# BUBLET/uav-airvision

Hardware: AMD Instinct MI355X
Metric: stereo frames/sec (LK+stereo+MSCKF-update) at 752x480 (higher is better)
Workload: dtype u8/int32 windows, f32 normal equations

## Files before the change

### uav_airvision_amd/csrc/lk.hip

```cpp
#include <math.h>
#include <stdio.h>
#include <stdlib.h>

#include "av_common.h"

namespace {

struct LKArgs {
    const uint8_t* pyrI;
    const uint8_t* pyrJ;
    int64_t stream_stride;
    PyrGeom g;
    const float* prev;
    float* next;
    uint8_t* status;
    const int* count;
    const int* index;
    int cap;
    int max_iter;
    double eps2;
    float min_eig_up, eps_lo, eps_hi;
    double min_eig;
    int n_set, gx;
    const uint8_t* imgI; const uint8_t* imgJ;
    int64_t imgI_stride, imgJ_stride;
    const int* mapI; const int* mapJ;
    unsigned long long* prof;
};

enum { LKP_HEAD = 0, LKP_ISTAGE, LKP_SETUP, LKP_JSTAGE, LKP_ITER, LKP_N, LKP_WAVES = LKP_N, LKP_ITERS, LKP_RESTAGES, LKP_LEVELS, LKP_SLOTS };

__device__ __forceinline__ void wave_lds_sync()
{
    __builtin_amdgcn_fence(__ATOMIC_RELEASE, "wavefront");
    __builtin_amdgcn_wave_barrier();
    __builtin_amdgcn_fence(__ATOMIC_ACQUIRE, "wavefront");
}

#define AV_DESCALE(x, n) (((x) + (1 << ((n)-1))) >> (n))

typedef short av_v2s __attribute__((ext_vector_type(2)));
__device__ __forceinline__ int dot2(uint32_t a, uint32_t b, int c)
{
    return __builtin_amdgcn_sdot2(__builtin_bit_cast(av_v2s, a), __builtin_bit_cast(av_v2s, b), c, false);
}
__device__ __forceinline__ int dot2_keep(uint32_t a, uint32_t b, int c)
{
    int r;
    asm("v_dot2_i32_i16 %0, %1, %2, %3" : "=v"(r) : "v"(a), "v"(b), "v"(c));
    return r;
}
__device__ __forceinline__ uint32_t pack16(int lo, int hi) { return ((uint32_t)lo & 0xFFFFu) | ((uint32_t)hi << 16); }

constexpr int TILE_ROWS = 24;
constexpr int TILE_COLS = 32;
constexpr int TPITCH = 36;
constexpr int TILE_DWORDS = 240;

typedef unsigned short av_v2u __attribute__((ext_vector_type(2)));

__device__ __forceinline__ uint32_t pk_add(uint32_t a, uint32_t b) { return __builtin_bit_cast(uint32_t, __builtin_bit_cast(av_v2u, a) + __builtin_bit_cast(av_v2u, b)); }
__device__ __forceinline__ uint32_t pk_sub(uint32_t a, uint32_t b) { return __builtin_bit_cast(uint32_t, __builtin_bit_cast(av_v2u, a) - __builtin_bit_cast(av_v2u, b)); }
__device__ __forceinline__ uint32_t pk_mul(uint32_t a, unsigned short k) { av_v2u kk = {k, k}; return __builtin_bit_cast(uint32_t, __builtin_bit_cast(av_v2u, a) * kk); }
// ... 160 lines not shown
        const bool rowin = (unsigned)(ipy + r) < (unsigned)h;
#pragma unroll
        for (int k = 0; k < 8; ++k) {
            const uint32_t m0 = (rowin && (unsigned)(ipx_o + 2 * k) < (unsigned)w) ? 0xFFFFu : 0u;
            const uint32_t m1 = (rowin && (unsigned)(ipx_o + 2 * k + 1) < (unsigned)w) ? 0xFFFF0000u : 0u;
            gxp[2 * k] &= (m0 | m1); gyp[2 * k] &= (m0 | m1);
        }
    }
#pragma unroll
    for (int k = 0; k < 7; ++k) {
        gxp[2 * k + 1] = mid(gxp[2 * k], gxp[2 * k + 2]);
        gyp[2 * k + 1] = mid(gyp[2 * k], gyp[2 * k + 2]);
    }
    const int rnd_i = 1 << (W_BITS - 6), rnd_d = 1 << (W_BITS - 1);
    int ixv[WIN + 1], iyv[WIN + 1];
    ixv[WIN] = 0; iyv[WIN] = 0;
#pragma unroll
    for (int c = 0; c < WIN; c += 5) {
        bilin5_seed(px[c], px[c + 1], px[c + 2], px[c + 3], px[c + 4], wtop, wbot, rnd_i, iv[c], iv[c + 1], iv[c + 2], iv[c + 3], iv[c + 4]);
        bilin5<W_BITS>(gxp[c], gxp[c + 1], gxp[c + 2], gxp[c + 3], gxp[c + 4], wtop, wbot, rnd_d, ixv[c], ixv[c + 1], ixv[c + 2], ixv[c + 3], ixv[c + 4]);
        bilin5<W_BITS>(gyp[c], gyp[c + 1], gyp[c + 2], gyp[c + 3], gyp[c + 4], wtop, wbot, rnd_d, iyv[c], iyv[c + 1], iyv[c + 2], iyv[c + 3], iyv[c + 4]);
    }
#pragma unroll
    for (int p = 0; p < (WIN + 1) / 2; ++p) {
        ixx[p] = __builtin_amdgcn_perm((uint32_t)ixv[2 * p + 1], (uint32_t)ixv[2 * p], 0x05040100u);
        iyy[p] = __builtin_amdgcn_perm((uint32_t)iyv[2 * p + 1], (uint32_t)iyv[2 * p], 0x05040100u);
        a11 = dot2(ixx[p], ixx[p], a11);
        a12 = dot2(ixx[p], iyy[p], a12);
        a22 = dot2(iyy[p], iyy[p], a22);
    }
    if (r >= WIN) { a11 = 0; a12 = 0; a22 = 0; }
}

template <int WIN, int OCC, bool PROF = false, int PTS = 16>
__device__ __forceinline__ bool lk_track_g16_body(const LKArgs& a)
{
    static_assert(WIN == 15, "lane map is built for the reference's 15x15 window");
    constexpr int W_BITS = 14;
    __shared__ uint32_t tile_all[PTS][TILE_DWORDS];
    unsigned pt[LKP_N] = {0, 0, 0, 0, 0}, plast = 0;
    unsigned pn_iter = 0, pn_restage = 0, pn_level = 0;
    unsigned long long rt0 = 0;
    if (PROF) { rt0 = __builtin_amdgcn_s_memrealtime(); plast = (unsigned)__builtin_readcyclecounter(); }
#define LK_STAMP(ph) do { if (PROF) { const unsigned t_ = (unsigned)__builtin_readcyclecounter(); pt[ph] += t_ - plast; plast = t_; } } while (0)
    const int g = threadIdx.x >> 4;
    const int r = threadIdx.x & 15;
    uint32_t* tile = tile_all[g];
    int s, bx;
    if (a.gx > 0) { const int L = blockIdx.x, j = L >> 3; s = (L & 7) + 8 * (j / a.gx); bx = j % a.gx; if (s >= a.n_set) return false; }
    else { s = blockIdx.y; bx = blockIdx.x; }
    const int slot = bx * PTS + g;
    const int sI = a.mapI ? a.mapI[s] : s, sJ = a.mapJ ? a.mapJ[s] : s;
    if (sI < 0 || sJ < 0) return false;
    const bool direct = a.index == nullptr && slot < a.cap;
    float prevx0 = 0.f, prevy0 = 0.f, curx = 0.f, cury = 0.f;
    if (direct) {
        const size_t p0 = (size_t)s * a.cap + slot;
        prevx0 = a.prev[2 * p0]; prevy0 = a.prev[2 * p0 + 1]; curx = a.next[2 * p0]; cury = a.next[2 * p0 + 1];
    }
    const int n = min(a.count[s], a.cap);
    if (slot >= n) return false;
    const int pidx = a.index ? a.index[(size_t)s * a.cap + slot] : slot;

    const uint8_t* PI = a.pyrI + sI * a.stream_stride;
    const uint8_t* PJ = a.pyrJ + sJ * a.stream_stride;
    const size_t pi = (size_t)s * a.cap + pidx;
    if (!direct) { prevx0 = a.prev[2 * pi]; prevy0 = a.prev[2 * pi + 1]; curx = a.next[2 * pi]; cury = a.next[2 * pi + 1]; }
    const float halfWin = (WIN - 1) * 0.5f;
    const bool rowact = r < WIN;
    bool ok = true;
    const uint32_t sel0 = 0x0C010C00u, sel1 = 0x0C020C01u, sel2 = 0x0C030C02u, sel3 = 0x0C040C03u;

    for (int level = a.g.levels - 1; level >= 0; --level) {
        const int w = a.g.w[level], h = a.g.h[level], pitch = a.g.pitch[level];
        const int col_lo = -AV_PYR_BORDER, col_hi = pitch - AV_PYR_BORDER;
        const float scale = __int_as_float((127 - level) << 23);
        float pvx = prevx0 * scale, pvy = prevy0 * scale;
        if (level == a.g.levels - 1) { curx = curx * scale; cury = cury * scale; }
        else                         { curx = curx * 2.f;   cury = cury * 2.f; }
        pvx -= halfWin; pvy -= halfWin;
        const int ipx = (int)floorf(pvx), ipy = (int)floorf(pvy);
        if (ipx < -WIN || ipx >= w || ipy < -WIN || ipy >= h) {
            if (level == 0) ok = false;
            continue;
        }
        float fa = pvx - ipx, fb = pvy - ipy;
        int iw00 = __float2int_rn((1.f - fa) * (1.f - fb) * (1 << W_BITS));
        int iw01 = __float2int_rn(fa * (1.f - fb) * (1 << W_BITS));
        int iw10 = __float2int_rn((1.f - fa) * fb * (1 << W_BITS));
        int iw11 = (1 << W_BITS) - iw00 - iw01 - iw10;
        uint32_t wtop = pack16(iw00, iw01), wbot = pack16(iw10, iw11);

        const int sub = r >> 3, dwl = r & 7;
        const uint32_t tofs = (uint32_t)(sub * (TPITCH / 4) + dwl);
// ... 26 lines not shown
                    uint32_t v = 0;
#pragma unroll 1
                    for (int bb = 0; bb < nbyte; ++bb) v |= (uint32_t)row[av_reflect101(xb + bb, w)] << (8 * bb);
                    tile[tofs + 2 * k * (TPITCH / 4)] = v;
                }
            }
        }
        wave_lds_sync();
        LK_STAMP(LKP_ISTAGE);

        int iv[WIN];
        uint32_t ixx[(WIN + 1) / 2], iyy[(WIN + 1) / 2];
        int a11, a12, a22;
        lk_patch_rows<WIN>([&](int t, uint32_t (&B)[5]) {
                               const uint32_t* rowp = tile + __mul24(r + t, TPITCH / 4);
#pragma unroll
                               for (int k = 0; k < 5; ++k) B[k] = rowp[k];
                           }, wtop, wbot, ipx, ipy, w, h, r, iv, ixx, iyy, a11, a12, a22);
        const float A11 = row_sum16_scaled(a11);
        const float A12 = row_sum16_scaled(a12);
        const float A22 = row_sum16_scaled(a22);
        float D = A11 * A22 - A12 * A12;
        const float minEig = (A22 + A11 - sqrtf((A11 - A22) * (A11 - A22) + 4.f * A12 * A12)) / (float)(2 * WIN * WIN);
        if (minEig < a.min_eig_up || D < 1.1920928955078125e-7f) {
            if (level == 0) ok = false;
            continue;
        }
        D = 1.f / D;

        float wx = curx - halfWin, wy = cury - halfWin;
        float pdx = 0.f, pdy = 0.f;
        int X0 = 0, Y0 = 0;
        bool staged = false;
        LK_STAMP(LKP_SETUP);
        for (int j = 0; j < a.max_iter; ++j) {
            if (PROF) ++pn_iter;
            const int inx = (int)floorf(wx), iny = (int)floorf(wy);
            if (inx < -WIN || inx >= w || iny < -WIN || iny >= h) {
                if (level == 0) ok = false;
                break;
            }
            int dx0 = inx - X0, dy0 = iny - Y0;
            if (!staged || (unsigned)dx0 > (unsigned)(TILE_COLS - 17) || (unsigned)dy0 > (unsigned)(TILE_ROWS - 16)) {
                X0 = min(max((inx - 6) & ~3, col_lo), col_hi - TILE_COLS);
                Y0 = min(max(iny - 4, -AV_PYR_BORDER), h + AV_PYR_BORDER - TILE_ROWS);
                LK_STAMP(LKP_ITER);
                if (PROF) ++pn_restage;
                wave_lds_sync();
                {
                    const bool extJ = level == 0 && a.imgJ != nullptr;
                    const uint8_t* LJ0 = extJ ? a.imgJ + (size_t)sJ * (size_t)a.imgJ_stride : PJ + a.g.off[level];
                    const int pJ = extJ ? w : pitch, bJ = extJ ? 0 : AV_PYR_BORDER;
                    if (!extJ || (X0 >= 0 && X0 + TILE_COLS <= w && Y0 >= 0 && Y0 + TILE_ROWS <= h)) {
                        const uint32_t joff = (uint32_t)(__mul24(Y0 + sub + bJ, pJ) + X0 + bJ + 4 * dwl);
                        uint32_t sv[TILE_ROWS / 2];
#pragma unroll
                        for (int k = 0; k < TILE_ROWS / 2; ++k)
                            sv[k] = *reinterpret_cast<const u32_unaligned*>(LJ0 + (size_t)(2 * k) * (size_t)pJ + joff);
#pragma unroll
                        for (int k = 0; k < TILE_ROWS / 2; ++k) tile[tofs + 2 * k * (TPITCH / 4)] = sv[k];
                    } else {
#pragma unroll 1
                        for (int k = 0; k < TILE_ROWS / 2; ++k) {
                            const uint8_t* row = LJ0 + (size_t)av_reflect101(Y0 + sub + 2 * k, h) * (size_t)w;
                            uint32_t v = 0;
#pragma unroll 1
// ... 21 lines not shown
            const uint32_t T2 = __builtin_amdgcn_alignbyte(d3, d2, sh), T3 = __builtin_amdgcn_alignbyte(d4, d3, sh);
            int df[WIN];
            jdiff5<0>(T0, T1, T2, T3, sel0, sel1, sel2, sel3, wtop, wbot, iv[0], iv[1], iv[2], iv[3], iv[4], df[0], df[1], df[2], df[3], df[4]);
            jdiff5<5>(T0, T1, T2, T3, sel0, sel1, sel2, sel3, wtop, wbot, iv[5], iv[6], iv[7], iv[8], iv[9], df[5], df[6], df[7], df[8], df[9]);
            jdiff5<10>(T0, T1, T2, T3, sel0, sel1, sel2, sel3, wtop, wbot, iv[10], iv[11], iv[12], iv[13], iv[14], df[10], df[11], df[12], df[13], df[14]);
            int b1 = 0, b2 = 0;
#pragma unroll
            for (int p = 0; p < (WIN + 1) / 2; ++p) {
                const uint32_t dp = 2 * p + 1 < WIN ? __builtin_amdgcn_perm((uint32_t)df[2 * p + 1 < WIN ? 2 * p + 1 : 0], (uint32_t)df[2 * p], 0x05040100u) : (uint32_t)df[2 * p];
                b1 = dot2(dp, ixx[p], b1);
                b2 = dot2(dp, iyy[p], b2);
            }
            if (!rowact) { b1 = 0; b2 = 0; }
            const float fb1 = row_sum16_scaled(b1);
            const float fb2 = row_sum16_scaled(b2);
            const float dx = (A12 * fb2 - A22 * fb1) * D;
            const float dy = (A12 * fb1 - A11 * fb2) * D;
            wx += dx; wy += dy;
            curx = wx + halfWin; cury = wy + halfWin;
            const float e32 = __builtin_fmaf(dx, dx, dy * dy);
            bool conv = e32 <= a.eps_lo;
            if (__builtin_amdgcn_ballot_w64(e32 > a.eps_lo && e32 < a.eps_hi) != 0) {
                asm volatile("; fp64 step test");
                conv = (double)dx * dx + (double)dy * dy <= a.eps2;
            }
            if (conv) break;
            if (j > 0 && fabsf(dx + pdx) <= 0.01f && fabsf(dy + pdy) <= 0.01f) {
                curx -= dx * 0.5f; cury -= dy * 0.5f;
                break;
            }
            pdx = dx; pdy = dy;
        }
        LK_STAMP(LKP_ITER);
    }
    if (r == 0) {
        a.next[2 * pi] = curx;
        a.next[2 * pi + 1] = cury;
        a.status[pi] = ok ? 1 : 0;
    }
    if (PROF) {
        LK_STAMP(LKP_HEAD);
        unsigned wi = pn_iter, wr = pn_restage, wl = pn_level;
#pragma unroll
        for (int d = 16; d < 64; d <<= 1) { wi = max(wi, (unsigned)__shfl_xor((int)wi, d, 64)); wr = max(wr, (unsigned)__shfl_xor((int)wr, d, 64)); wl = max(wl, (unsigned)__shfl_xor((int)wl, d, 64)); }
        const bool book = blockIdx.x % 61 == 0;
        if (book && (threadIdx.x & 63) == 0) {
            for (int k = 0; k < LKP_N; ++k) atomicAdd(a.prof + k, (unsigned long long)pt[k]);
            atomicAdd(a.prof + LKP_WAVES, 1ull);
            atomicAdd(a.prof + LKP_SLOTS + 3, __builtin_amdgcn_s_memrealtime() - rt0);
            atomicAdd(a.prof + LKP_ITERS, (unsigned long long)wi);
            atomicAdd(a.prof + LKP_RESTAGES, (unsigned long long)wr);
            atomicAdd(a.prof + LKP_LEVELS, (unsigned long long)wl);
        }
        if (book && r == 0) { atomicAdd(a.prof + LKP_SLOTS, 1ull); atomicAdd(a.prof + LKP_SLOTS + 1, (unsigned long long)pn_iter); atomicAdd(a.prof + LKP_SLOTS + 2, (unsigned long long)pn_restage); }
    }
#undef LK_STAMP
    return true;
}

template <int WIN> __global__ __launch_bounds__(64, 5) void lk_track_g16_kernel(LKArgs a) { lk_track_g16_body<WIN, 5, false, 4>(a); }
template <int WIN> __global__ __launch_bounds__(256, 5) void lk_track_g16_w4_kernel(LKArgs a) { lk_track_g16_body<WIN, 5>(a); }
template <int WIN> __global__ __launch_bounds__(256, 5) void lk_track_g16_prof_kernel(LKArgs a) { lk_track_g16_body<WIN, 5, true>(a); }

static unsigned long long* g_lk_prof = nullptr;
static void lk_prof_report()
{
    if (!g_lk_prof) return;
    unsigned long long h[LKP_SLOTS + 4];
    if (hipDeviceSynchronize() != hipSuccess || hipMemcpy(h, g_lk_prof, sizeof(h), hipMemcpyDeviceToHost) != hipSuccess) return;
    static const char* names[LKP_N] = {"head+tail", "I staging", "set-up", "J staging", "iterations"};
    double tot = 0;
    for (int k = 0; k < LKP_N; ++k) tot += (double)h[k];
    const double nw = (double)h[LKP_WAVES];
    fprintf(stderr, "AV_LK_PROF: %.0f wavefronts booked (one workgroup in 61), %.0f s_memtime ticks per wavefront = %.1f us on the 100 MHz clock: %.0f ticks per us\n",
            nw, tot / nw, (double)h[LKP_SLOTS + 3] / nw / 100., tot / ((double)h[LKP_SLOTS + 3] / 100.));
    for (int k = 0; k < LKP_N; ++k) fprintf(stderr, "AV_LK_PROF:   %-10s %8.0f ticks per wavefront  %5.1f %%\n", names[k], (double)h[k] / nw, 100. * (double)h[k] / tot);
    fprintf(stderr, "AV_LK_PROF: per wavefront (max over its 4 points): %.2f levels, %.2f iterations, %.2f J stagings; per point: %.2f iterations, %.2f J stagings\n",
            (double)h[LKP_LEVELS] / nw, (double)h[LKP_ITERS] / nw, (double)h[LKP_RESTAGES] / nw,
            (double)h[LKP_SLOTS + 1] / (double)h[LKP_SLOTS], (double)h[LKP_SLOTS + 2] / (double)h[LKP_SLOTS]);
}


constexpr int LKG_MAX_WIN = 31, LKG_PER_LANE = (LKG_MAX_WIN * LKG_MAX_WIN + 63) / 64;

__device__ __forceinline__ long long wave_sum_i64(long long v)
{
#pragma unroll
    for (int d = 32; d >= 1; d >>= 1) v += __shfl_xor(v, d, 64);
    return v;
}

struct LKLevel { const uint8_t* base; int pitch, w, h; };
__device__ __forceinline__ int lkg_pix(const LKLevel& L, int x, int y) { return L.base[(size_t)av_reflect101_any(y, L.h) * L.pitch + av_reflect101_any(x, L.w)]; }

__global__ __launch_bounds__(256) void lk_track_generic_kernel(LKArgs a, int WIN)
{
    constexpr int W_BITS = 14;
    const int lane = threadIdx.x & 63;
    const int s = blockIdx.y, slot = blockIdx.x * 4 + (threadIdx.x >> 6);
    const int sI = a.mapI ? a.mapI[s] : s, sJ = a.mapJ ? a.mapJ[s] : s;
    if (sI < 0 || sJ < 0) return;
    const int n = min(a.count[s], a.cap);
    if (slot >= n) return;
    const int pidx = a.index ? a.index[(size_t)s * a.cap + slot] : slot;
    const size_t pi = (size_t)s * a.cap + pidx;
    const float prevx0 = a.prev[2 * pi], prevy0 = a.prev[2 * pi + 1];
    float curx = a.next[2 * pi], cury = a.next[2 * pi + 1];
    const float halfWin = (WIN - 1) * 0.5f;
    const int win2 = WIN * WIN;
    const double FLT_SCALE_D = 1.0 / (1 << 20);
    bool ok = true;
    for (int level = a.g.levels - 1; level >= 0; --level) {
// ... 106 lines not shown
        a.next[2 * pi + 1] = cury;
        a.status[pi] = ok ? 1 : 0;
    }
}

}

static int lk_fill_args(LKArgs& a, const uint8_t* pyrI, const uint8_t* pyrJ, int64_t stream_stride, const PyrGeom& g,
                        const float* prev, float* next, uint8_t* status, const int* count, int cap,
                        const LKParams& p, const int* index,
                        const uint8_t* imgI, int64_t imgI_stride, const uint8_t* imgJ, int64_t imgJ_stride, const int* mapI, const int* mapJ)
{
    if (p.win < 3 || p.win > LKG_MAX_WIN) { av_set_error("av_lk_track: winSize %d outside 3 .. %d", p.win, LKG_MAX_WIN); return AV_E_INVALID; }
    a.pyrI = pyrI; a.pyrJ = pyrJ; a.stream_stride = stream_stride; a.g = g;
    for (int l = 1; l < a.g.levels; ++l)
        if (a.g.w[l] <= p.win || a.g.h[l] <= p.win) { a.g.levels = l; break; }
    a.prev = prev; a.next = next; a.status = status; a.count = count; a.index = index; a.cap = cap;
    a.max_iter = p.max_iter; a.eps2 = p.eps2;
    a.min_eig_up = (float)p.min_eig;
    if ((double)a.min_eig_up < p.min_eig) a.min_eig_up = nextafterf(a.min_eig_up, INFINITY);
    if (p.eps2 >= 1e-30) { a.eps_lo = (float)(p.eps2 * (1. - 0x1p-18)); a.eps_hi = (float)(p.eps2 * (1. + 0x1p-18)); }
    else { a.eps_lo = -1.f; a.eps_hi = INFINITY; }
    a.min_eig = p.min_eig;
    a.imgI = imgI; a.imgJ = imgJ; a.imgI_stride = imgI_stride; a.imgJ_stride = imgJ_stride; a.mapI = mapI; a.mapJ = mapJ; a.prof = nullptr;
    a.n_set = 0; a.gx = 0;
    return AV_OK;
}

static bool lk_prof_on()
{
    static const bool prof = [] {
        const char* e = getenv("AV_LK_PROF");
        if (!(e && atoi(e) == 1)) return false;
        if (hipMalloc(&g_lk_prof, sizeof(unsigned long long) * (LKP_SLOTS + 4)) != hipSuccess) { g_lk_prof = nullptr; return false; }
        (void)hipMemset(g_lk_prof, 0, sizeof(unsigned long long) * (LKP_SLOTS + 4));
        (void)hipDeviceSynchronize();
        atexit(lk_prof_report);
        return true;
    }();
    return prof;
}

static dim3 lk_g16_grid(LKArgs& a, int n_set, int launch_pts, int pts_per_wg)
{
    static const bool xcd_map = [] { const char* e = getenv("AV_LK_XCD"); return !(e && atoi(e) == 0); }();
    const int gx = (launch_pts + pts_per_wg - 1) / pts_per_wg;
    a.n_set = n_set; a.gx = xcd_map ? gx : 0;
    return xcd_map ? dim3((unsigned)gx * 8u * (unsigned)((n_set + 7) / 8)) : dim3(gx, n_set);
}

int av_launch_lk(const uint8_t* pyrI, const uint8_t* pyrJ, int64_t stream_stride, int n_set, const PyrGeom& g,
                 const float* prev, float* next, uint8_t* status, const int* count, int cap, int launch_pts,
                 const LKParams& p, hipStream_t st, const int* index,
                 const uint8_t* imgI, int64_t imgI_stride, const uint8_t* imgJ, int64_t imgJ_stride, const int* mapI, const int* mapJ)
{
    if (n_set <= 0 || launch_pts <= 0) return AV_OK;
    LKArgs a;
    int rc = lk_fill_args(a, pyrI, pyrJ, stream_stride, g, prev, next, status, count, cap, p, index, imgI, imgI_stride, imgJ, imgJ_stride, mapI, mapJ);
    if (rc) return rc;
    if (launch_pts > cap) launch_pts = cap;
    if (p.win != 15) {
        a.n_set = n_set; a.gx = 0;
        hipLaunchKernelGGL(lk_track_generic_kernel, dim3((launch_pts + 3) / 4, n_set), dim3(256), 0, st, a, p.win);
        AV_LAUNCH_CHECK();
        return AV_OK;
    }
    const bool prof = lk_prof_on();
    static const bool w1 = [] { const char* e = getenv("AV_LK_WG"); return !(e && atoi(e) == 256); }();
    const int wgp = (prof || !w1) ? 256 : 64;
    const dim3 grid = lk_g16_grid(a, n_set, launch_pts, wgp / 16);
    a.prof = g_lk_prof;
    if (prof) hipLaunchKernelGGL(lk_track_g16_prof_kernel<15>, grid, dim3(256), 0, st, a);
    else if (wgp == 64) hipLaunchKernelGGL(lk_track_g16_kernel<15>, grid, dim3(64), 0, st, a);
    else hipLaunchKernelGGL(lk_track_g16_w4_kernel<15>, grid, dim3(256), 0, st, a);
    AV_LAUNCH_CHECK();
    return AV_OK;
}

AV_EXPORT int av_lk_track(const uint8_t* pyrI_dev, const uint8_t* pyrJ_dev, int64_t pyr_stride, int n_set,
                          int w, int h, int levels,
                          const float* prev_dev, float* next_dev, uint8_t* status_dev, const int32_t* count_dev, int cap,
                          int win, int max_iter, double eps, double min_eig_threshold, void* stream)
{
    av_pyr_layout lay;
    int rc = av_pyramid_layout(w, h, levels, &lay);
    if (rc) return rc;
    if (!pyrI_dev || !pyrJ_dev || !prev_dev || !next_dev || !status_dev || !count_dev || cap <= 0 || n_set < 0 ||
        pyr_stride < lay.bytes) {
        av_set_error("av_lk_track: bad arguments");
        return AV_E_INVALID;
    }
    LKParams p;
    p.win = win;
    p.max_iter = max_iter < 0 ? 0 : (max_iter > 100 ? 100 : max_iter);
    double e = eps < 0 ? 0. : (eps > 10. ? 10. : eps);
    p.eps2 = e * e;
    p.min_eig = min_eig_threshold;
    return av_launch_lk(pyrI_dev, pyrJ_dev, pyr_stride, n_set, av_make_geom(lay), prev_dev, next_dev, status_dev,
                        count_dev, cap, cap, p, (hipStream_t)stream, nullptr);
}
// ... 1 lines not shown
```

Before: 200,400.

## Track each LK point with 8 lanes handling two window rows each

After: 198,800 (median of 2 runs). No clear change (-0.8%).

```diff
diff --git a/uav_airvision_amd/csrc/lk.hip b/uav_airvision_amd/csrc/lk.hip
--- a/uav_airvision_amd/csrc/lk.hip
+++ b/uav_airvision_amd/csrc/lk.hip
@@ -29,6 +29,8 @@
 };
 
 enum { LKP_HEAD = 0, LKP_ISTAGE, LKP_SETUP, LKP_JSTAGE, LKP_ITER, LKP_N, LKP_WAVES = LKP_N, LKP_ITERS, LKP_RESTAGES, LKP_LEVELS, LKP_SLOTS };
+enum { LKP_DIV4 = LKP_SLOTS + 4, LKP_NDIV4, LKP_DIV8, LKP_NDIV8, LKP_WORDS };
+constexpr int LKD_G4 = 8, LKD_G8 = 4, LKD_WORDS = (LKD_G4 + LKD_G8) * (AV_MAX_LEVELS + 1);
 
 __device__ __forceinline__ void wave_lds_sync()
 {
@@ -255,8 +257,39 @@
     if (r >= WIN) { a11 = 0; a12 = 0; a22 = 0; }
 }
 
+__device__ __forceinline__ void lk_div_active(unsigned* lvm, int g)
+{
+    atomicMax(lvm + (LKD_G4 + LKD_G8) * AV_MAX_LEVELS + (g >> 2), 1u);
+    atomicMax(lvm + (LKD_G4 + LKD_G8) * AV_MAX_LEVELS + LKD_G4 + (g >> 3), 1u);
+}
+__device__ __forceinline__ void lk_div_level(unsigned* lvm, int g, int level, unsigned iters)
+{
+    atomicMax(lvm + (g >> 2) * AV_MAX_LEVELS + level, iters);
+    atomicMax(lvm + (LKD_G4 + (g >> 3)) * AV_MAX_LEVELS + level, iters);
+}
+__device__ __forceinline__ void lk_div_init(unsigned* lvm)
+{
+    for (int i = threadIdx.x; i < LKD_WORDS; i += blockDim.x) lvm[i] = 0;
+    __syncthreads();
+}
+__device__ __forceinline__ void lk_div_book(const LKArgs& a, const unsigned* lvm)
+{
+    __syncthreads();
+    if (threadIdx.x != 0 || blockIdx.x % 61 != 0) return;
+    unsigned long long it[2] = {0, 0}, ng[2] = {0, 0};
+    for (int k = 0; k < 2; ++k)
+        for (int grp = 0; grp < (k ? LKD_G8 : LKD_G4); ++grp) {
+            const int row = (k ? LKD_G4 : 0) + grp;
+            if (!lvm[(LKD_G4 + LKD_G8) * AV_MAX_LEVELS + row]) continue;
+            ++ng[k];
+            for (int l = 0; l < AV_MAX_LEVELS; ++l) it[k] += lvm[row * AV_MAX_LEVELS + l];
+        }
+    atomicAdd(a.prof + LKP_DIV4, it[0]); atomicAdd(a.prof + LKP_NDIV4, ng[0]);
+    atomicAdd(a.prof + LKP_DIV8, it[1]); atomicAdd(a.prof + LKP_NDIV8, ng[1]);
+}
+
 template <int WIN, int OCC, bool PROF = false, int PTS = 16>
-__device__ __forceinline__ bool lk_track_g16_body(const LKArgs& a)
+__device__ __forceinline__ bool lk_track_g16_body(const LKArgs& a, unsigned* lvm = nullptr)
 {
     static_assert(WIN == 15, "lane map is built for the reference's 15x15 window");
     constexpr int W_BITS = 14;
@@ -283,6 +316,7 @@
     }
     const int n = min(a.count[s], a.cap);
     if (slot >= n) return false;
+    if (PROF && r == 0) lk_div_active(lvm, g);
     const int pidx = a.index ? a.index[(size_t)s * a.cap + slot] : slot;
 
     const uint8_t* PI = a.pyrI + sI * a.stream_stride;
@@ -375,6 +409,7 @@
         float pdx = 0.f, pdy = 0.f;
         int X0 = 0, Y0 = 0;
         bool staged = false;
+        const unsigned it_lv0 = pn_iter;
         LK_STAMP(LKP_SETUP);
         for (int j = 0; j < a.max_iter; ++j) {
             if (PROF) ++pn_iter;
@@ -462,6 +497,7 @@
             pdx = dx; pdy = dy;
         }
         LK_STAMP(LKP_ITER);
+        if (PROF && r == 0) lk_div_level(lvm, g, level, pn_iter - it_lv0);
     }
     if (r == 0) {
         a.next[2 * pi] = curx;
@@ -490,13 +526,438 @@
 
 template <int WIN> __global__ __launch_bounds__(64, 5) void lk_track_g16_kernel(LKArgs a) { lk_track_g16_body<WIN, 5, false, 4>(a); }
 template <int WIN> __global__ __launch_bounds__(256, 5) void lk_track_g16_w4_kernel(LKArgs a) { lk_track_g16_body<WIN, 5>(a); }
-template <int WIN> __global__ __launch_bounds__(256, 5) void lk_track_g16_prof_kernel(LKArgs a) { lk_track_g16_body<WIN, 5, true>(a); }
+template <int WIN> __global__ __launch_bounds__(256, 5) void lk_track_g16_prof_kernel(LKArgs a)
+{
+    __shared__ unsigned lvm[LKD_WORDS];
+    lk_div_init(lvm);
+    lk_track_g16_body<WIN, 5, true>(a, lvm);
+    lk_div_book(a, lvm);
+}
+
+constexpr int G8_TILE_DWORDS = 216;
+
+__device__ __forceinline__ float row_sum8_scaled(int v)
+{
+    v += __builtin_amdgcn_update_dpp(0, v, 0xB1, 0xF, 0xF, false);
+    int lo = v & 0xFFFF, hi = v >> 16;
+    lo += __builtin_amdgcn_update_dpp(0, lo, 0x4E, 0xF, 0xF, false);
+    hi += __builtin_amdgcn_update_dpp(0, hi, 0x4E, 0xF, 0xF, false);
+    lo += __builtin_amdgcn_update_dpp(0, lo, 0x141, 0xF, 0xF, false);
+    hi += __builtin_amdgcn_update_dpp(0, hi, 0x141, 0xF, 0xF, false);
+    return __builtin_fmaf((float)hi, 0x1p-4f, (float)lo * 0x1p-20f);
+}
+
+#define AV_G8_BILIN(X) AV_G8_BILIN_(X)
+#define AV_G8_BILIN_(BOT, TAIL)                                                                                                   \
+    "v_dot2_i32_i16 %0, %5, %15, %17\n\t" "v_dot2_i32_i16 %1, %6, %15, %17\n\t" "v_dot2_i32_i16 %2, %7, %15, %17\n\t"            \
+    "v_dot2_i32_i16 %3, %8, %15, %17\n\t" "v_dot2_i32_i16 %4, %9, %15, %17\n\t"                                                   \
+    "v_dot2c_i32_i16" BOT " %0, %10, %16" TAIL "\n\t" "v_dot2c_i32_i16" BOT " %1, %11, %16" TAIL "\n\t"                           \
+    "v_dot2c_i32_i16" BOT " %2, %12, %16" TAIL "\n\t" "v_dot2c_i32_i16" BOT " %3, %13, %16" TAIL "\n\t"                           \
+    "v_dot2c_i32_i16" BOT " %4, %14, %16" TAIL "\n\t"
+#define AV_G8_DPP "_dpp", " row_shl:1 row_mask:0xf bank_mask:0xf bound_ctrl:1"
+#define AV_G8_OWN "", ""
+template <int SH, bool NB>
+__device__ __forceinline__ void bilin5_2(const uint32_t* t, const uint32_t* b, uint32_t wtop, uint32_t wbot, int rnd, int* o)
+{
+#define AV_G8_SHIFT "v_ashrrev_i32 %0, %18, %0\n\tv_ashrrev_i32 %1, %18, %1\n\tv_ashrrev_i32 %2, %18, %2\n\tv_ashrrev_i32 %3, %18, %3\n\tv_ashrrev_i32 %4, %18, %4"
+#define AV_G8_ARGS : "=&v"(o[0]), "=&v"(o[1]), "=&v"(o[2]), "=&v"(o[3]), "=&v"(o[4]) \
+                   : "v"(t[0]), "v"(t[1]), "v"(t[2]), "v"(t[3]), "v"(t[4]), "v"(b[0]), "v"(b[1]), "v"(b[2]), "v"(b[3]), "v"(b[4]), \
+                     "v"(wtop), "v"(wbot), "v"(rnd)
+    if (NB) asm(AV_G8_BILIN(AV_G8_DPP) AV_G8_SHIFT AV_G8_ARGS, "n"(SH));
+    else    asm(AV_G8_BILIN(AV_G8_OWN) AV_G8_SHIFT AV_G8_ARGS, "n"(SH));
+#undef AV_G8_SHIFT
+}
+template <bool NB>
+__device__ __forceinline__ void bilin5_2_seed(const uint32_t* t, const uint32_t* b, uint32_t wtop, uint32_t wbot, int rnd, int* o)
+{
+#define AV_G8_SEED "v_and_b32 %0, %18, %0\n\tv_and_b32 %1, %18, %1\n\tv_and_b32 %2, %18, %2\n\tv_and_b32 %3, %18, %3\n\tv_and_b32 %4, %18, %4\n\t" \
+                   "v_sub_u32 %0, %19, %0\n\tv_sub_u32 %1, %19, %1\n\tv_sub_u32 %2, %19, %2\n\tv_sub_u32 %3, %19, %3\n\tv_sub_u32 %4, %19, %4"
+    if (NB) asm(AV_G8_BILIN(AV_G8_DPP) AV_G8_SEED AV_G8_ARGS, "s"(0xfffffe00u), "s"(0x100u));
+    else    asm(AV_G8_BILIN(AV_G8_OWN) AV_G8_SEED AV_G8_ARGS, "s"(0xfffffe00u), "s"(0x100u));
+#undef AV_G8_SEED
+}
+template <bool NB>
+__device__ __forceinline__ void jdot5_2(const uint32_t* t, const uint32_t* b, uint32_t wtop, uint32_t wbot, const int* s, int* d)
+{
+#define AV_G8_JD(X) AV_G8_JD_(X)
+#define AV_G8_JD_(BOT, TAIL)                                                                                                     \
+    "v_dot2_i32_i16 %0, %5, %15, %17\n\t" "v_dot2_i32_i16 %1, %6, %15, %18\n\t" "v_dot2_i32_i16 %2, %7, %15, %19\n\t"            \
+    "v_dot2_i32_i16 %3, %8, %15, %20\n\t" "v_dot2_i32_i16 %4, %9, %15, %21\n\t"                                                   \
+    "v_dot2c_i32_i16" BOT " %0, %10, %16" TAIL "\n\t" "v_dot2c_i32_i16" BOT " %1, %11, %16" TAIL "\n\t"                           \
+    "v_dot2c_i32_i16" BOT " %2, %12, %16" TAIL "\n\t" "v_dot2c_i32_i16" BOT " %3, %13, %16" TAIL "\n\t"                           \
+    "v_dot2c_i32_i16" BOT " %4, %14, %16" TAIL "\n\t"                                                                             \
+    "v_ashrrev_i32 %0, 9, %0\n\tv_ashrrev_i32 %1, 9, %1\n\tv_ashrrev_i32 %2, 9, %2\n\tv_ashrrev_i32 %3, 9, %3\n\tv_ashrrev_i32 %4, 9, %4"
+#define AV_G8_JARGS : "=&v"(d[0]), "=&v"(d[1]), "=&v"(d[2]), "=&v"(d[3]), "=&v"(d[4]) \
+                    : "v"(t[0]), "v"(t[1]), "v"(t[2]), "v"(t[3]), "v"(t[4]), "v"(b[0]), "v"(b[1]), "v"(b[2]), "v"(b[3]), "v"(b[4]), \
+                      "v"(wtop), "v"(wbot), "v"(s[0]), "v"(s[1]), "v"(s[2]), "v"(s[3]), "v"(s[4])
+    if (NB) asm(AV_G8_JD(AV_G8_DPP) AV_G8_JARGS);
+    else    asm(AV_G8_JD(AV_G8_OWN) AV_G8_JARGS);
+#undef AV_G8_JD
+#undef AV_G8_JD_
+#undef AV_G8_JARGS
+}
+#undef AV_G8_ARGS
+#undef AV_G8_BILIN
+#undef AV_G8_BILIN_
+#undef AV_G8_DPP
+#undef AV_G8_OWN
+
+template <int WIN>
+__device__ __forceinline__ void lk_patch_rows2(const uint32_t* rowp, uint32_t wtop, uint32_t wbot, uint32_t wtopB, uint32_t wbotB,
+                                               int ipx, int ipy, int w, int h, int q,
+                                               int (&ivA)[WIN], uint32_t (&ixxA)[(WIN + 1) / 2], uint32_t (&iyyA)[(WIN + 1) / 2],
+                                               int (&ivB)[WIN], uint32_t (&ixxB)[(WIN + 1) / 2], uint32_t (&iyyB)[(WIN + 1) / 2],
+                                               int& a11, int& a12, int& a22)
+{
+    constexpr int W_BITS = 14;
+    uint32_t E[4][9];
+#pragma unroll
+    for (int t = 0; t < 4; ++t) {
+        uint32_t B[5];
+#pragma unroll
+        for (int k = 0; k < 5; ++k) B[k] = rowp[t * (TPITCH / 4) + k];
+#pragma unroll
+        for (int k = 0; k < 9; ++k) {
+            const int b0 = 2 * k;
+            E[t][k] = __builtin_amdgcn_perm(0, B[b0 >> 2], 0x0C000C00u | (uint32_t)(b0 & 3) | ((uint32_t)((b0 & 3) + 1) << 16));
+        }
+    }
+    auto mid = [](uint32_t x, uint32_t y) -> uint32_t { return __builtin_amdgcn_perm(y, x, 0x05040302u); };
+    uint32_t pxA[WIN], pxB[WIN];
+#pragma unroll
+    for (int k = 0; k < 8; ++k) { pxA[2 * k] = mid(E[1][k], E[1][k + 1]); pxB[2 * k] = mid(E[2][k], E[2][k + 1]); }
+#pragma unroll
+    for (int k = 0; k < 7; ++k) { pxA[2 * k + 1] = E[1][k + 1]; pxB[2 * k + 1] = E[2][k + 1]; }
+    uint32_t gxA[WIN + 1], gyA[WIN + 1], gxB[WIN + 1], gyB[WIN + 1];
+#pragma unroll
+    for (int rr = 0; rr < 2; ++rr) {
+        uint32_t* gxp = rr ? gxB : gxA;
+        uint32_t* gyp = rr ? gyB : gyA;
+        uint32_t t0E[9], t1E[9];
+#pragma unroll
+        for (int k = 0; k < 9; ++k) {
+            t0E[k] = pk_add(pk_mul(pk_add(E[rr][k], E[rr + 2][k]), 3), pk_mul(E[rr + 1][k], 10));
+            t1E[k] = pk_sub(E[rr + 2][k], E[rr][k]);
+        }
+#pragma unroll
+        for (int k = 0; k < 8; ++k) {
+            gxp[2 * k] = pk_sub(t0E[k + 1], t0E[k]);
+            gyp[2 * k] = pk_add(pk_mul(pk_add(t1E[k + 1], t1E[k]), 3), pk_mul(mid(t1E[k], t1E[k + 1]), 10));
+        }
+    }
+    const bool inside = ipx >= 0 && ipx + WIN < w && ipy >= 0 && ipy + WIN < h;
+    if (__builtin_amdgcn_ballot_w64(!inside) != 0) {
+        int ipx_o = ipx;
+        asm volatile("" : "+v"(ipx_o));
+#pragma unroll
+        for (int rr = 0; rr < 2; ++rr) {
+            uint32_t* gxp = rr ? gxB : gxA;
+            uint32_t* gyp = rr ? gyB : gyA;
+            const bool rowin = (unsigned)(ipy + 2 * q + rr) < (unsigned)h;
+#pragma unroll
+            for (int k = 0; k < 8; ++k) {
+                const uint32_t m0 = (rowin && (unsigned)(ipx_o + 2 * k) < (unsigned)w) ? 0xFFFFu : 0u;
+                const uint32_t m1 = (rowin && (unsigned)(ipx_o + 2 * k + 1) < (unsigned)w) ? 0xFFFF0000u : 0u;
+                gxp[2 * k] &= (m0 | m1); gyp[2 * k] &= (m0 | m1);
+            }
+        }
+    }
+#pragma unroll
+    for (int k = 0; k < 7; ++k) {
+        gxA[2 * k + 1] = mid(gxA[2 * k], gxA[2 * k + 2]); gyA[2 * k + 1] = mid(gyA[2 * k], gyA[2 * k + 2]);
+        gxB[2 * k + 1] = mid(gxB[2 * k], gxB[2 * k + 2]); gyB[2 * k + 1] = mid(gyB[2 * k], gyB[2 * k + 2]);
+    }
+    const int rnd_i = 1 << (W_BITS - 6), rnd_d = 1 << (W_BITS - 1);
+    int ixA[WIN + 1], iyA[WIN + 1], ixB[WIN + 1], iyB[WIN + 1];
+    ixA[WIN] = 0; iyA[WIN] = 0; ixB[WIN] = 0; iyB[WIN] = 0;
+#pragma unroll
+    for (int c = 0; c < WIN; c += 5) {
+        bilin5_2_seed<false>(pxA + c, pxB + c, wtop, wbot, rnd_i, ivA + c);
+        bilin5_2_seed<true>(pxB + c, pxA + c, wtopB, wbotB, rnd_i, ivB + c);
+        bilin5_2<W_BITS, false>(gxA + c, gxB + c, wtop, wbot, rnd_d, ixA + c);
+        bilin5_2<W_BITS, true>(gxB + c, gxA + c, wtopB, wbotB, rnd_d, ixB + c);
+        bilin5_2<W_BITS, false>(gyA + c, gyB + c, wtop, wbot, rnd_d, iyA + c);
+        bilin5_2<W_BITS, true>(gyB + c, gyA + c, wtopB, wbotB, rnd_d, iyB + c);
+    }
+    a11 = 0; a12 = 0; a22 = 0;
+#pragma unroll
+    for (int p = 0; p < (WIN + 1) / 2; ++p) {
+        ixxA[p] = __builtin_amdgcn_perm((uint32_t)ixA[2 * p + 1], (uint32_t)ixA[2 * p], 0x05040100u);
+        iyyA[p] = __builtin_amdgcn_perm((uint32_t)iyA[2 * p + 1], (uint32_t)iyA[2 * p], 0x05040100u);
+        ixxB[p] = __builtin_amdgcn_perm((uint32_t)ixB[2 * p + 1], (uint32_t)ixB[2 * p], 0x05040100u);
+        iyyB[p] = __builtin_amdgcn_perm((uint32_t)iyB[2 * p + 1], (uint32_t)iyB[2 * p], 0x05040100u);
+        a11 = dot2(ixxA[p], ixxA[p], a11); a12 = dot2(ixxA[p], iyyA[p], a12); a22 = dot2(iyyA[p], iyyA[p], a22);
+        a11 = dot2(ixxB[p], ixxB[p], a11); a12 = dot2(ixxB[p], iyyB[p], a12); a22 = dot2(iyyB[p], iyyB[p], a22);
+    }
+}
+
+template <int WIN, bool PROF = false, int PTS = 8>
+__device__ __forceinline__ bool lk_track_g8_body(const LKArgs& a, unsigned* lvm = nullptr)
+{
+    static_assert(WIN == 15, "lane map is built for the reference's 15x15 window");
+    constexpr int W_BITS = 14;
+    __shared__ uint32_t tile_all[PTS][G8_TILE_DWORDS];
+    unsigned pt[LKP_N] = {0, 0, 0, 0, 0}, plast = 0;
+    unsigned pn_iter = 0, pn_restage = 0, pn_level = 0;
+    unsigned long long rt0 = 0;
+    if (PROF) { rt0 = __builtin_amdgcn_s_memrealtime(); plast = (unsigned)__builtin_readcyclecounter(); }
+#define LK_STAMP(ph) do { if (PROF) { const unsigned t_ = (unsigned)__builtin_readcyclecounter(); pt[ph] += t_ - plast; plast = t_; } } while (0)
+    const int g = threadIdx.x >> 3;
+    const int q = threadIdx.x & 7;
+    uint32_t* tile = tile_all[g];
+    int s, bx;
+    if (a.gx > 0) { const int L = blockIdx.x, j = L >> 3; s = (L & 7) + 8 * (j / a.gx); bx = j % a.gx; if (s >= a.n_set) return false; }
+    else { s = blockIdx.y; bx = blockIdx.x; }
+    const int slot = bx * PTS + g;
+    const int sI = a.mapI ? a.mapI[s] : s, sJ = a.mapJ ? a.mapJ[s] : s;
+    if (sI < 0 || sJ < 0) return false;
+    const bool direct = a.index == nullptr && slot < a.cap;
+    float prevx0 = 0.f, prevy0 = 0.f, curx = 0.f, cury = 0.f;
+    if (direct) {
+        const size_t p0 = (size_t)s * a.cap + slot;
+        prevx0 = a.prev[2 * p0]; prevy0 = a.prev[2 * p0 + 1]; curx = a.next[2 * p0]; cury = a.next[2 * p0 + 1];
+    }
+    const int n = min(a.count[s], a.cap);
+    if (slot >= n) return false;
+    if (PROF && q == 0) lk_div_active(lvm, g);
+    const int pidx = a.index ? a.index[(size_t)s * a.cap + slot] : slot;
+
+    const uint8_t* PI = a.pyrI + sI * a.stream_stride;
+    const uint8_t* PJ = a.pyrJ + sJ * a.stream_stride;
+    const size_t pi = (size_t)s * a.cap + pidx;
+    if (!direct) { prevx0 = a.prev[2 * pi]; prevy0 = a.prev[2 * pi + 1]; curx = a.next[2 * pi]; cury = a.next[2 * pi + 1]; }
+    const float halfWin = (WIN - 1) * 0.5f;
+    const bool rowBin = q < 7;
+    bool ok = true;
+    const uint32_t sel0 = 0x0C010C00u, sel1 = 0x0C020C01u, sel2 = 0x0C030C02u, sel3 = 0x0C040C03u;
+    typedef uint32_t __attribute__((aligned(1))) u32_unaligned;
+
+    for (int level = a.g.levels - 1; level >= 0; --level) {
+        const int w = a.g.w[level], h = a.g.h[level], pitch = a.g.pitch[level];
+        const int col_lo = -AV_PYR_BORDER, col_hi = pitch - AV_PYR_BORDER;
+        const float scale = __int_as_float((127 - level) << 23);
+        float pvx = prevx0 * scale, pvy = prevy0 * scale;
+        if (level == a.g.levels - 1) { curx = curx * scale; cury = cury * scale; }
+        else                         { curx = curx * 2.f;   cury = cury * 2.f; }
+        pvx -= halfWin; pvy -= halfWin;
+        const int ipx = (int)floorf(pvx), ipy = (int)floorf(pvy);
+        if (ipx < -WIN || ipx >= w || ipy < -WIN || ipy >= h) {
+            if (level == 0) ok = false;
+            continue;
+        }
+        float fa = pvx - ipx, fb = pvy - ipy;
+        int iw00 = __float2int_rn((1.f - fa) * (1.f - fb) * (1 << W_BITS));
+        int iw01 = __float2int_rn(fa * (1.f - fb) * (1 << W_BITS));
+        int iw10 = __float2int_rn((1.f - fa) * fb * (1 << W_BITS));
+        int iw11 = (1 << W_BITS) - iw00 - iw01 - iw10;
+        uint32_t wtop = pack16(iw00, iw01), wbot = pack16(iw10, iw11);
+
+        LK_STAMP(LKP_HEAD);
+        if (PROF) ++pn_level;
+        wave_lds_sync();
+        {
+            const bool extI = level == 0 && a.imgI != nullptr;
+            const uint8_t* L0 = extI ? a.imgI + (size_t)sI * (size_t)a.imgI_stride : PI + a.g.off[level];
+            const int pI = extI ? w : pitch, bI = extI ? 0 : AV_PYR_BORDER;
+            const bool act = q < 5;
+            if (!extI || (ipx >= 1 && ipx + 16 < w && ipy >= 1 && ipy + 16 < h)) {
+                const uint32_t loff = (uint32_t)(__mul24(ipy - 1 + bI, pI) + (ipx - 1 + bI) + (q < 4 ? 4 * q : 14));
+                const uint32_t shamt = q == 4 ? 16u : 0u;
+                uint32_t sv[18];
+#pragma unroll
+                for (int k = 0; k < 18; ++k) {
+                    sv[k] = 0;
+                    if (act) sv[k] = *reinterpret_cast<const u32_unaligned*>(L0 + (size_t)k * (size_t)pI + loff);
+                }
+#pragma unroll
+                for (int k = 0; k < 18; ++k)
+                    if (act) tile[q + k * (TPITCH / 4)] = sv[k] >> shamt;
+            } else if (act) {
+                const int xb = ipx - 1 + (q < 4 ? 4 * q : 16), nbyte = q < 4 ? 4 : 2;
+#pragma unroll 1
+                for (int k = 0; k < 18; ++k) {
+                    const uint8_t* row = L0 + (size_t)av_reflect101(ipy - 1 + k, h) * (size_t)w;
+                    uint32_t v = 0;
+#pragma unroll 1
+                    for (int bb = 0; bb < nbyte; ++bb) v |= (uint32_t)row[av_reflect101(xb + bb, w)] << (8 * bb);
+                    tile[q + k * (TPITCH / 4)] = v;
+                }
+            }
+        }
+        wave_lds_sync();
+        LK_STAMP(LKP_ISTAGE);
+
+        int ivA[WIN], ivB[WIN];
+        uint32_t ixxA[(WIN + 1) / 2], iyyA[(WIN + 1) / 2], ixxB[(WIN + 1) / 2], iyyB[(WIN + 1) / 2];
+        int a11, a12, a22;
+        lk_patch_rows2<WIN>(tile + 2 * q * (TPITCH / 4), wtop, wbot, rowBin ? wtop : 0u, rowBin ? wbot : 0u, ipx, ipy, w, h, q,
+                            ivA, ixxA, iyyA, ivB, ixxB, iyyB, a11, a12, a22);
+        const float A11 = row_sum8_scaled(a11);
+        const float A12 = row_sum8_scaled(a12);
+        const float A22 = row_sum8_scaled(a22);
+        float D = A11 * A22 - A12 * A12;
+        const float minEig = (A22 + A11 - sqrtf((A11 - A22) * (A11 - A22) + 4.f * A12 * A12)) / (float)(2 * WIN * WIN);
+        if (minEig < a.min_eig_up || D < 1.1920928955078125e-7f) {
+            if (level == 0) ok = false;
+            continue;
+        }
+        D = 1.f / D;
+
+        float wx = curx - halfWin, wy = cury - halfWin;
+        float pdx = 0.f, pdy = 0.f;
+        int X0 = 0, Y0 = 0;
+        bool staged = false;
+        const unsigned it_lv0 = pn_iter;
+        LK_STAMP(LKP_SETUP);
+        for (int j = 0; j < a.max_iter; ++j) {
+            if (PROF) ++pn_iter;
+            const int inx = (int)floorf(wx), iny = (int)floorf(wy);
+            if (inx < -WIN || inx >= w || iny < -WIN || iny >= h) {
+                if (level == 0) ok = false;
+                break;
+            }
+            int dx0 = inx - X0, dy0 = iny - Y0;
+            if (!staged || (unsigned)dx0 > (unsigned)(TILE_COLS - 17) || (unsigned)dy0 > (unsigned)(TILE_ROWS - 16)) {
+                X0 = min(max((inx - 6) & ~3, col_lo), col_hi - TILE_COLS);
+                Y0 = min(max(iny - 4, -AV_PYR_BORDER), h + AV_PYR_BORDER - TILE_ROWS);
+                LK_STAMP(LKP_ITER);
+                if (PROF) ++pn_restage;
+                wave_lds_sync();
+                {
+                    const bool extJ = level == 0 && a.imgJ != nullptr;
+                    const uint8_t* LJ0 = extJ ? a.imgJ + (size_t)sJ * (size_t)a.imgJ_stride : PJ + a.g.off[level];
+                    const int pJ = extJ ? w : pitch, bJ = extJ ? 0 : AV_PYR_BORDER;
+                    if (!extJ || (X0 >= 0 && X0 + TILE_COLS <= w && Y0 >= 0 && Y0 + TILE_ROWS <= h)) {
+                        const uint32_t joff = (uint32_t)(__mul24(Y0 + bJ, pJ) + X0 + bJ + 4 * q);
+#pragma unroll
+                        for (int hh = 0; hh < 2; ++hh) {
+                            uint32_t sv[TILE_ROWS / 2];
+#pragma unroll
+                            for (int k = 0; k < TILE_ROWS / 2; ++k)
+                                sv[k] = *reinterpret_cast<const u32_unaligned*>(LJ0 + (size_t)(k + hh * (TILE_ROWS / 2)) * (size_t)pJ + joff);
+#pragma unroll
+                            for (int k = 0; k < TILE_ROWS / 2; ++k) tile[q + (k + hh * (TILE_ROWS / 2)) * (TPITCH / 4)] = sv[k];
+                        }
+                    } else {
+#pragma unroll 1
+                        for (int k = 0; k < TILE_ROWS; ++k) {
+                            const uint8_t* row = LJ0 + (size_t)av_reflect101(Y0 + k, h) * (size_t)w;
+                            uint32_t v = 0;
+#pragma unroll 1
+                            for (int bb = 0; bb < 4; ++bb) v |= (uint32_t)row[av_reflect101(X0 + 4 * q + bb, w)] << (8 * bb);
+                            tile[q + k * (TPITCH / 4)] = v;
+                        }
+                    }
+                }
+                wave_lds_sync();
+                LK_STAMP(LKP_JSTAGE);
+                staged = true;
+                dx0 = inx - X0; dy0 = iny - Y0;
+            }
+            fa = wx - inx; fb = wy - iny;
+            iw00 = __float2int_rn((1.f - fa) * (1.f - fb) * (1 << W_BITS));
+            iw01 = __float2int_rn(fa * (1.f - fb) * (1 << W_BITS));
+            iw10 = __float2int_rn((1.f - fa) * fb * (1 << W_BITS));
+            iw11 = (1 << W_BITS) - iw00 - iw01 - iw10;
+            wtop = pack16(iw00, iw01); wbot = pack16(iw10, iw11);
+
+            const int sh = dx0 & 3;
+            const uint32_t* rp = tile + __mul24(dy0 + 2 * q, TPITCH / 4) + (dx0 >> 2);
+            uint32_t TA[4], TB[4];
+            {
+                const uint32_t d0 = rp[0], d1 = rp[1], d2 = rp[2], d3 = rp[3], d4 = rp[4];
+                TA[0] = __builtin_amdgcn_alignbyte(d1, d0, sh); TA[1] = __builtin_amdgcn_alignbyte(d2, d1, sh);
+                TA[2] = __builtin_amdgcn_alignbyte(d3, d2, sh); TA[3] = __builtin_amdgcn_alignbyte(d4, d3, sh);
+                const uint32_t e0 = rp[9], e1 = rp[10], e2 = rp[11], e3 = rp[12], e4 = rp[13];
+                TB[0] = __builtin_amdgcn_alignbyte(e1, e0, sh); TB[1] = __builtin_amdgcn_alignbyte(e2, e1, sh);
+                TB[2] = __builtin_amdgcn_alignbyte(e3, e2, sh); TB[3] = __builtin_amdgcn_alignbyte(e4, e3, sh);
+            }
+            int b1 = 0, b2 = 0;
+            int cA = 0, cB = 0;
+#pragma unroll
+            for (int c0 = 0; c0 < WIN; c0 += 5) {
+                uint32_t pA[5], pB[5];
+#pragma unroll
+                for (int i = 0; i < 5; ++i) {
+                    const int c = c0 + i, dq = c >> 2, o = c & 3;
+                    const uint32_t sl = o == 0 ? sel0 : o == 1 ? sel1 : o == 2 ? sel2 : sel3;
+                    pA[i] = __builtin_amdgcn_perm(TA[dq < 3 ? dq + 1 : 3], TA[dq], sl);
+                    pB[i] = __builtin_amdgcn_perm(TB[dq < 3 ? dq + 1 : 3], TB[dq], sl);
+                }
+                int dA[5], dB[5];
+                jdot5_2<false>(pA, pB, wtop, wbot, ivA + c0, dA);
+                jdot5_2<true>(pB, pA, wtop, wbot, ivB + c0, dB);
+#pragma unroll
+                for (int i = 0; i < 5; ++i) {
+                    const int c = c0 + i;
+                    if ((c & 1) == 0 && c + 1 < WIN) { cA = dA[i]; cB = dB[i]; continue; }
+                    const uint32_t dpA = c & 1 ? __builtin_amdgcn_perm((uint32_t)dA[i], (uint32_t)cA, 0x05040100u) : (uint32_t)dA[i];
+                    const uint32_t dpB = c & 1 ? __builtin_amdgcn_perm((uint32_t)dB[i], (uint32_t)cB, 0x05040100u) : (uint32_t)dB[i];
+                    b1 = dot2(dpA, ixxA[c >> 1], b1); b2 = dot2(dpA, iyyA[c >> 1], b2);
+                    b1 = dot2(dpB, ixxB[c >> 1], b1); b2 = dot2(dpB, iyyB[c >> 1], b2);
+                }
+            }
+            const float fb1 = row_sum8_scaled(b1);
+            const float fb2 = row_sum8_scaled(b2);
+            const float dx = (A12 * fb2 - A22 * fb1) * D;
+            const float dy = (A12 * fb1 - A11 * fb2) * D;
+            wx += dx; wy += dy;
+            curx = wx + halfWin; cury = wy + halfWin;
+            const float e32 = __builtin_fmaf(dx, dx, dy * dy);
+            bool conv = e32 <= a.eps_lo;
+            if (__builtin_amdgcn_ballot_w64(e32 > a.eps_lo && e32 < a.eps_hi) != 0) {
+                asm volatile("; fp64 step test");
+                conv = (double)dx * dx + (double)dy * dy <= a.eps2;
+            }
+            if (conv) break;
+            if (j > 0 && fabsf(dx + pdx) <= 0.01f && fabsf(dy + pdy) <= 0.01f) {
+                curx -= dx * 0.5f; cury -= dy * 0.5f;
+                break;
+            }
+            pdx = dx; pdy = dy;
+        }
+        LK_STAMP(LKP_ITER);
+        if (PROF && q == 0) lk_div_level(lvm, g, level, pn_iter - it_lv0);
+    }
+    if (q == 0) {
+        a.next[2 * pi] = curx;
+        a.next[2 * pi + 1] = cury;
+        a.status[pi] = ok ? 1 : 0;
+    }
+    if (PROF) {
+        LK_STAMP(LKP_HEAD);
+        unsigned wi = pn_iter, wr = pn_restage, wl = pn_level;
+#pragma unroll
+        for (int d = 8; d < 64; d <<= 1) { wi = max(wi, (unsigned)__shfl_xor((int)wi, d, 64)); wr = max(wr, (unsigned)__shfl_xor((int)wr, d, 64)); wl = max(wl, (unsigned)__shfl_xor((int)wl, d, 64)); }
+        const bool book = blockIdx.x % 61 == 0;
+        if (book && (threadIdx.x & 63) == 0) {
+            for (int k = 0; k < LKP_N; ++k) atomicAdd(a.prof + k, (unsigned long long)pt[k]);
+            atomicAdd(a.prof + LKP_WAVES, 1ull);
+            atomicAdd(a.prof + LKP_SLOTS + 3, __builtin_amdgcn_s_memrealtime() - rt0);
+            atomicAdd(a.prof + LKP_ITERS, (unsigned long long)wi);
+            atomicAdd(a.prof + LKP_RESTAGES, (unsigned long long)wr);
+            atomicAdd(a.prof + LKP_LEVELS, (unsigned long long)wl);
+        }
+        if (book && q == 0) { atomicAdd(a.prof + LKP_SLOTS, 1ull); atomicAdd(a.prof + LKP_SLOTS + 1, (unsigned long long)pn_iter); atomicAdd(a.prof + LKP_SLOTS + 2, (unsigned long long)pn_restage); }
+    }
+#undef LK_STAMP
+    return true;
+}
+
+template <int WIN, int OCC> __global__ __launch_bounds__(64, OCC) void lk_track_g8_kernel(LKArgs a) { lk_track_g8_body<WIN>(a); }
+template <int WIN> __global__ __launch_bounds__(256, 4) void lk_track_g8_prof_kernel(LKArgs a)
+{
+    __shared__ unsigned lvm[LKD_WORDS];
+    lk_div_init(lvm);
+    lk_track_g8_body<WIN, true, 32>(a, lvm);
+    lk_div_book(a, lvm);
+}
 
 static unsigned long long* g_lk_prof = nullptr;
 static void lk_prof_report()
 {
     if (!g_lk_prof) return;
-    unsigned long long h[LKP_SLOTS + 4];
+    unsigned long long h[LKP_WORDS];
     if (hipDeviceSynchronize() != hipSuccess || hipMemcpy(h, g_lk_prof, sizeof(h), hipMemcpyDeviceToHost) != hipSuccess) return;
     static const char* names[LKP_N] = {"head+tail", "I staging", "set-up", "J staging", "iterations"};
     double tot = 0;
@@ -508,6 +969,9 @@
     fprintf(stderr, "AV_LK_PROF: per wavefront (max over its 4 points): %.2f levels, %.2f iterations, %.2f J stagings; per point: %.2f iterations, %.2f J stagings\n",
             (double)h[LKP_LEVELS] / nw, (double)h[LKP_ITERS] / nw, (double)h[LKP_RESTAGES] / nw,
             (double)h[LKP_SLOTS + 1] / (double)h[LKP_SLOTS], (double)h[LKP_SLOTS + 2] / (double)h[LKP_SLOTS]);
+    fprintf(stderr, "AV_LK_PROF: iterations per point pass (sum over levels of the per-level maximum): %.2f for 4 consecutive points "
+            "(%.0f groups), %.2f for 8 (%.0f groups)\n",
+            (double)h[LKP_DIV4] / (double)h[LKP_NDIV4], (double)h[LKP_NDIV4], (double)h[LKP_DIV8] / (double)h[LKP_NDIV8], (double)h[LKP_NDIV8]);
 }
 
 
@@ -680,8 +1144,8 @@
     static const bool prof = [] {
         const char* e = getenv("AV_LK_PROF");
         if (!(e && atoi(e) == 1)) return false;
-        if (hipMalloc(&g_lk_prof, sizeof(unsigned long long) * (LKP_SLOTS + 4)) != hipSuccess) { g_lk_prof = nullptr; return false; }
-        (void)hipMemset(g_lk_prof, 0, sizeof(unsigned long long) * (LKP_SLOTS + 4));
+        if (hipMalloc(&g_lk_prof, sizeof(unsigned long long) * LKP_WORDS) != hipSuccess) { g_lk_prof = nullptr; return false; }
+        (void)hipMemset(g_lk_prof, 0, sizeof(unsigned long long) * LKP_WORDS);
         (void)hipDeviceSynchronize();
         atexit(lk_prof_report);
         return true;
@@ -714,6 +1178,17 @@
         return AV_OK;
     }
     const bool prof = lk_prof_on();
+    const char* lanes = getenv("AV_LK_LANES");
+    if (!(lanes && atoi(lanes) == 16)) {
+        static const bool occ5 = [] { const char* e = getenv("AV_LK_G8_OCC"); return e && atoi(e) == 5; }();
+        const dim3 grid = lk_g16_grid(a, n_set, launch_pts, prof ? 32 : 8);
+        a.prof = g_lk_prof;
+        if (prof) hipLaunchKernelGGL(lk_track_g8_prof_kernel<15>, grid, dim3(256), 0, st, a);
+        else if (occ5) hipLaunchKernelGGL((lk_track_g8_kernel<15, 5>), grid, dim3(64), 0, st, a);
+        else hipLaunchKernelGGL((lk_track_g8_kernel<15, 4>), grid, dim3(64), 0, st, a);
+        AV_LAUNCH_CHECK();
+        return AV_OK;
+    }
     static const bool w1 = [] { const char* e = getenv("AV_LK_WG"); return !(e && atoi(e) == 256); }();
     const int wgp = (prof || !w1) ? 256 : 64;
     const dim3 grid = lk_g16_grid(a, n_set, launch_pts, wgp / 16);
```
